# CVlab315/Domain-Adaptative-Hand-Pose-Estimation

Hardware: AMD Instinct MI355X
Metric: images/sec (unique source+target images per A+B+C training iteration, 2*B*N/t_iter) (higher is better)
Workload: dtype bf16; 1 GPU; RHD->H3D domain-adaptation iteration (steps A+B+C), resnet50 + 3-deconv neck + main head + 3 adversarial multiscale-fusion heads, 256x256, batch 64 source + 64 target per GPU, random init, synthetic batches; arch=resnet50, image_size=256, per_gpu_batch=64, global_batch=64, parallelism=dp1, hip_graphs=True, gradient_exchange=none (one rank)

## Files before the change

### domain-adaptative-hand-pose-estimation_amd/build.py

```python
import os
import re
import shutil
import subprocess
import sys
import tempfile
from concurrent.futures import ThreadPoolExecutor

HERE = os.path.dirname(os.path.abspath(__file__))
CSRC = os.path.join(HERE, 'csrc')
OUT = os.path.join(HERE, 'libmi355pose.so')
SOURCES = ['api.hip', 'igemm.hip', 'pgemm.hip', 'igemm_fp8.hip', 'mx_fp8.hip', 'wgrad_fp8.hip', 'bn.hip', 'pool_layout.hip', 'pw21.hip', 'heatmap.hip', 'optim.hip', 'augment.hip', 'teacher.hip', 'eval.hip', 'mmd.hip', 'jfa.hip', 'proto.hip', 'mixup.hip']
HEADERS = ['common.h', 'conv_plan.h', 'igemm_common.h', 'fp8_common.h', 'joint_pool.h', 'adam_slice.h']
HIPCC = os.environ.get('HIPCC', '/opt/rocm/bin/hipcc')
LLVM_BIN = os.environ.get('MI355_LLVM_BIN', '/opt/rocm/lib/llvm/bin')
FLAGS = ['--offload-arch=gfx950', '-O3', '-std=c++17', '-fPIC', '-Wall', '-Wno-unused-function',
         '-ffp-contract=off',
         '-fno-slp-vectorize']

_PK = re.compile(r'\bv_pk_[a-z0-9_]+_f32\b')
_OPSEL = re.compile(r'\bop_sel:\[([01,]+)\]')
_OPSEL_HI = re.compile(r'\bop_sel_hi:\[([01,]+)\]')


def _negated(flag):
    if flag.startswith('-fno-'):
        return '-f' + flag[5:]
# ... 132 lines not shown
```

### domain-adaptative-hand-pose-estimation_amd/csrc/conv_plan.h

```cpp
#pragma once
#include <stdlib.h>
#include "common.h"

#define MAX_TAPS 52
struct Tap { int8_t dy, dx; int16_t widx; };

struct Phase { int OHp, OWp, out_oy, out_ox, M, ntaps, tap0, ntm; };
struct GatherArgs {
  const void* A; const void* B; void* D;
  const float* bias; const void* residual; const float* scale;
  int Hi, Wi, Ci;
  int in_sy, in_sx;
  int Ho, Wo;
  int out_sy, out_sx;
  int Nout, ldb, ldd;
  int cshift;
  int accumulate;
  int nphase, ntn, ntiles;
  int hw;
  int lw;
  unsigned a_bytes, b_bytes;
  size_t stat_bytes;
  int stat_slices;
  const void* bnb_x; const void* bnb_y;
// ... 40 lines not shown
  bool stats256 = conv_knob("MI355_STATS_256", 1) != 0;
  int phases = (int)conv_knob("MI355_PHASES", 1);
  int wg_blocks = (int)conv_knob("MI355_WG_BLOCKS", 768);
  int wgrad_kw = (int)conv_knob("MI355_WGRAD_KW", 1);
  int wgrad_kw2 = (int)conv_knob("MI355_WGRAD_KW2", 1);
  bool wgrad_group256 = conv_knob("MI355_WGRAD_GROUP256", 1) != 0;
  bool wgrad_kw_group = conv_knob("MI355_WGRAD_KW_GROUP", 1) != 0;
  int wg_group_blocks = (int)conv_knob("MI355_WG_GROUP_BLOCKS", 512);
  int wg_group256_blocks = (int)conv_knob("MI355_WG_GROUP256_BLOCKS", 256);
  int wg_kw_group_blocks = (int)conv_knob("MI355_WG_KW_GROUP_BLOCKS", 512);
  int pgemm = (int)conv_knob("MI355_PGEMM", 1), pgemm_set = -1;
  int pg_add_maxk = (int)conv_knob("MI355_PG_ADD", 1) * 64;
  long pg_min_rows = conv_knob("MI355_PG_MIN_ROWS", 32768);
  int pg_ring = (int)conv_knob("MI355_PG_RING", 0), pg_bm = (int)conv_knob("MI355_PG_BM", 64);
  int pg_per_cu = (int)conv_knob("MI355_PG_PER_CU", 2);
  int fp8_tile = (int)conv_knob("MI355_FP8_TILE", -1);
  long fp8_kw3 = conv_knob("MI355_FP8_KW3", 1024), fp8_kw3_set = -1;
};
inline ConvKnobs& conv_knobs() { static ConvKnobs k; return k; }

static inline void describe_fwd(GatherArgs& a, const mi355_conv_desc* d) {
  a.Hi = d->Hi; a.Wi = d->Wi; a.Ci = d->Ci; a.in_sy = a.in_sx = d->stride;
  a.Ho = d->Ho; a.Wo = d->Wo; a.out_sy = a.out_sx = 1;
  a.Nout = d->Co; a.ldd = d->Co; a.ldb = d->kh * d->kw * d->Ci;
  a.nphase = 1; a.ph[0].OHp = d->Ho; a.ph[0].OWp = d->Wo; a.ph[0].M = d->N * d->Ho * d->Wo; a.ph[0].ntaps = d->kh * d->kw;
  for (int i = 0; i < d->kh; ++i)
    for (int j = 0; j < d->kw; ++j) { Tap& t = a.taps[i * d->kw + j]; t.dy = (int8_t)(i - d->pad); t.dx = (int8_t)(j - d->pad); t.widx = (int16_t)(i * d->kw + j); }
}
static inline bool describe_dgrad(GatherArgs& a, const mi355_conv_desc* d) {
  const int s = d->stride;
// ... 18 lines not shown
        for (int kw = 0; kw < d->kw; ++kw) {
          if ((px + d->pad - kw) % s != 0) continue;
          Tap& t = a.taps[nt++]; t.dy = (int8_t)((py + d->pad - kh) / s); t.dx = (int8_t)((px + d->pad - kw) / s);
          t.widx = (int16_t)(kh * d->kw + kw);
        }
      }
      P.ntaps = nt - P.tap0;
      if (P.ntaps == 0) continue;
      ++a.nphase;
    }
  return need_zero;
}
static inline bool dgrad_fuses_stats(const GatherArgs& a, int stride, bool need_zero) { return !need_zero && a.nphase == stride * stride; }
static inline size_t conv_stats_bytes(long rows, int C) { return (size_t)(rows / 64 + 8) * C * 3 * sizeof(float); }

enum ConvFamily { CONV_GATHER = 0, CONV_PGEMM, CONV_FP8, CONV_MX };
struct ConvBuild {
  int family = CONV_GATHER;
  int bm = 64, bn = 64;
  bool f32 = false;
  bool small_c = false;
  bool hm = false;
  bool dma = false;
  bool kw3 = false;
  bool cat = false;
  int kg = 1;
  int ns = 0; bool add = false;
  bool bf8 = false;
  int epi = 0;
};
static inline void conv_build_text(const ConvBuild& b, char* out, size_t n) {
  char epi[8] = "";
  if (b.epi) snprintf(epi, sizeof(epi), " epi%d", b.epi);
  if (b.family == CONV_PGEMM) snprintf(out, n, "pgemm bm%d bn%d ns%d%s%s", b.bm, b.bn, b.ns, epi, b.add ? " add" : "");
  else if (b.family == CONV_GATHER)
    snprintf(out, n, "%sg%dx%d%s%s%s%s%s%s%s", b.cat ? "cat " : "", b.bm, b.bn, b.f32 ? " f32" : "", b.small_c ? " small" : "", b.hm ? " hm" : "",
             b.dma ? " dma" : "", b.kw3 ? " kw3" : "", b.kg == 2 ? " kg2" : "", epi);
  else snprintf(out, n, "%s g%dx%d%s%s%s", b.family == CONV_MX ? "mx" : "f8", b.bm, b.bn, b.kw3 ? " kw3" : "", b.bf8 ? " bf8" : "", epi);
}

static inline bool kw3_shape(const GatherArgs& a) {
  if (!(a.nphase == 1 && a.ph[0].ntaps == 9 && a.in_sx == 1 && a.in_sy == 1 && a.out_sx == 1 && a.out_sy == 1 &&
        a.ph[0].OWp == a.Wi && a.ph[0].OHp == a.Hi && a.Wo == a.Wi && a.Ho == a.Hi && a.Wi >= 8 && a.Wi <= 128 && ilog2_exact(a.Wi) >= 0))
    return false;
  for (int g = 0; g < 3; ++g) {
    const Tap* tp = a.taps + a.ph[0].tap0 + 3 * g;
    int seen = 0;
    for (int k = 0; k < 3; ++k) { if (tp[k].dy != tp[0].dy || tp[k].dx < -1 || tp[k].dx > 1) return false; seen |= 1 << (tp[k].dx + 1); }
    if (seen != 7 || tp[0].dy < -1 || tp[0].dy > 1) return false;
// ... 89 lines not shown
  return b;
}
static inline int pgemm_plan_grid(GatherArgs& a, ConvBuild& b) {
  const int nk = a.Ci >> 6;
  a.pg_nadd = pgemm_nadd(b.ns, nk, b.add);
  const int smem = pgemm_smem(b.bm, b.bn, b.ns, nk, a.pg_nadd);
  if (smem > 160 * 1024) return 0;
  const int ntm = a.ph[0].ntm = cdiv(a.ph[0].M, b.bm);
  a.ntn = cdiv(a.Nout, b.bn);
  a.ntiles = ntm * a.ntn; a.stat_slices = 0;
  if (a.stat_partial && (b.add || (size_t)ntm * a.Nout * 3 * sizeof(float) > a.stat_bytes)) a.stat_partial = nullptr;
  b.epi = a.stat_partial ? 1 : 0;
  return smem;
}

static inline ConvBuild choose_conv(const GatherArgs& a, int elem_size, const ConvKnobs& k) {
  if (a.A2) return choose_cat(a, elem_size, k);
  const bool bf16 = elem_size == 2;
  if (bf16 && pgemm_eligible(a, 2, k)) return choose_pgemm(a, k);
  const GatherWork w = gather_work(a, elem_size);
  ConvBuild b;
  b.f32 = !bf16;
  if (w.small) { b.bm = 128; b.small_c = true; return b; }
  if (k.tile >= 0 && k.tile <= 3) {
    static const int forced[4][2] = {{128, 128}, {64, 128}, {128, 64}, {64, 64}};
    b.bm = forced[k.tile][0]; b.bn = forced[k.tile][1];
    return b;
  }
  const bool kw3 = k.kw3 && bf16 && kw3_shape(a) && (a.Nout > 64 || (k.kw3_n64 && a.Nout == 64)) && a.Ci % 64 == 0 && !a.bnb_partial;
  const long rows128 = cdiv(w.Mtot, 128L);
  if (a.Nout <= 64) {
    if (kw3 && (rows128 >= 2048 || k.kw3 == 2)) { b.bm = 128; b.kw3 = true; }
    else if (rows128 >= 512) b.bm = 128;
  }
// ... 178 lines not shown
```

### domain-adaptative-hand-pose-estimation_amd/csrc/igemm.hip

```cpp
#include "common.h"
#include <stdlib.h>

#include "igemm_common.h"

template <typename T> struct MmaTraits;
template <> struct MmaTraits<bf16_t> { static constexpr int BK = 64; static constexpr int CH = 8; };
template <> struct MmaTraits<float> { static constexpr int BK = 32; static constexpr int CH = 4; };

#define GATHER_STAGES 1
template <typename T, int BM, int BN, int STAGES = 1, bool KW3 = false>
struct GatherSmem {
  static constexpr int kARows = KW3 ? BM + 4 * (BM / 8) + 4 : BM;
  static constexpr int kStage = (kARows + BN) * 128;
  static constexpr int kOutStride = BN * (int)sizeof(T) + 16;
  static constexpr int kOut = BM * kOutStride;
  static constexpr int kBytes = (STAGES * kStage > kOut ? STAGES * kStage : kOut) + BM * 4;
};

template <typename T, int BM, int BN, bool SMALL_C, int WGM = 2, int WGN = 2, bool HM_OUT = false, bool DMA = false, int EPI = 0,
          bool KW3 = false, bool CAT = false, int KG = 1>
__global__ __launch_bounds__(64 * WGM * WGN * KG, (KW3 && BM == 256) ? 2 : 1) void gather_gemm_kernel(const GatherArgs p) {
  constexpr int CH = MmaTraits<T>::CH;
  constexpr int GTHR = 64 * WGM * WGN;
  constexpr int NTHR = GTHR * KG, RPP = GTHR / 8;
// ... 1308 lines not shown
    flops += 2.0 * a.ph[i].M * (double)a.Nout * a.ph[i].ntaps * a.Ci;
  }
  {
    const long imgs = a.ph[0].M / ((long)a.ph[0].OHp * a.ph[0].OWp);
    a.a_bytes = (unsigned)(imgs * a.Hi * a.Wi * a.Ci * (long)sizeof(T));
    a.b_bytes = (unsigned)((long)a.Nout * a.ldb * (long)sizeof(T));
  }
  if (a.A2) flops += 2.0 * Mtot * (double)a.Nout * a.c2;
  ProfScope ps(st, flops, (double)a.a_bytes + (double)a.b_bytes * ntaps_tot / (a.ldb / a.Ci) + (double)Mtot * a.Nout * sizeof(T) +
                              (a.A2 ? (double)a.a2_bytes + a.b2_bytes : 0.0));
  if (a.A2) {
    if ((a.Ci / CH) < 8 || a.nphase != 1 || a.out_sx != 1 || a.out_sy != 1 || a.bnb_partial || a.residual || a.accumulate)
      MI_FAIL(MI355_EINVAL, "concat-K forward: plain single-phase forward conv with >= 8 input chunks only");
    if (a.c2 < CH || a.c2 % CH || a.c2 > MmaTraits<T>::BK) MI_FAIL(MI355_EINVAL, "concat-K forward: c2=%d must be a multiple of %d and <= %d", a.c2, CH, MmaTraits<T>::BK);
  }
  const ConvBuild b = choose_conv(a, (int)sizeof(T), conv_knobs());
  if (b.family == CONV_PGEMM) return launch_pgemm_build(a, b, st);
  if (!launch_gather_build<T>(a, b, st)) MI_FAIL(MI355_EINVAL, "gather: no such build (%dx%d)", b.bm, b.bn);
  MI_CHECK_LAUNCH(b.cat ? "gather_gemm_cat" : "gather_gemm");
  return MI355_OK;
}

static int check_desc(const mi355_conv_desc* d, bool crop_ok = false) {
  if (!d) MI_FAIL(MI355_EINVAL, "null conv desc");
  if (d->dtype != MI355_F32 && d->dtype != MI355_BF16 && d->dtype != MI355_FP8) MI_FAIL(MI355_EINVAL, "bad dtype %d", d->dtype);
  if (d->kh * d->kw > MAX_TAPS || d->kh < 1 || d->kw < 1) MI_FAIL(MI355_EINVAL, "unsupported kernel %dx%d", d->kh, d->kw);
  if (d->stride < 1 || d->stride > 2) MI_FAIL(MI355_EINVAL, "unsupported stride %d", d->stride);
  const int fho = (d->Hi + 2 * d->pad - d->kh) / d->stride + 1, fwo = (d->Wi + 2 * d->pad - d->kw) / d->stride + 1;
  const bool cropped = crop_ok && d->stride == 1 && d->kh > 1 && d->dtype != MI355_FP8 && d->Ho >= 1 && d->Wo >= 1 && d->Ho <= fho && d->Wo <= fwo;
  if (!cropped && (d->Ho != fho || d->Wo != fwo))
    MI_FAIL(MI355_EINVAL, "conv desc: output size %dx%d inconsistent with input %dx%d k%d s%d p%d", d->Ho, d->Wo, d->Hi, d->Wi, d->kh, d->stride, d->pad);
  const long esz = d->dtype == MI355_F32 ? 4 : 2;
// ... 491 lines not shown
```

### domain-adaptative-hand-pose-estimation_amd/csrc/igemm_common.h

```cpp
#pragma once
#include "common.h"
#include "conv_plan.h"

template <typename T> __device__ __forceinline__ uint4 keep_masked(uint4 q, unsigned mb) {
  unsigned w[4] = {q.x, q.y, q.z, q.w};
  if constexpr (sizeof(T) == 2) {
#pragma unroll
    for (int i = 0; i < 4; ++i)
      w[i] &= ((0u - ((mb >> (2 * i)) & 1u)) & 0x0000ffffu) | ((0u - ((mb >> (2 * i + 1)) & 1u)) & 0xffff0000u);
  } else {
#pragma unroll
    for (int i = 0; i < 4; ++i) w[i] &= 0u - ((mb >> i) & 1u);
  }
  return make_uint4(w[0], w[1], w[2], w[3]);
}

__device__ __forceinline__ int swz128(int r, int c) { return r * 128 + ((c ^ ((r >> 1) & 7)) << 4); }

__device__ __forceinline__ int xcd_remap(int bid, int nblk) {
  int q = nblk >> 3, r = nblk & 7, x = bid & 7, i = bid >> 3;
  int start = (x < r) ? x * (q + 1) : r * (q + 1) + (x - r) * q;
  return start + i;
}

typedef __attribute__((ext_vector_type(4))) unsigned int u32x4_t;
#define OOB_OFF ((int)0x80000000)
__device__ __forceinline__ __amdgpu_buffer_rsrc_t make_rsrc(const void* p, unsigned bytes) {
  return __builtin_amdgcn_make_buffer_rsrc(const_cast<void*>(p), 0, bytes, 0x00020000);
}
__device__ __forceinline__ uint4 buf_load16(__amdgpu_buffer_rsrc_t rs, int byte_off) {
  u32x4_t v = __builtin_amdgcn_raw_buffer_load_b128(rs, byte_off, 0, 0);
  return make_uint4(v[0], v[1], v[2], v[3]);
}
__device__ __forceinline__ unsigned buf_load4(__amdgpu_buffer_rsrc_t rs, int byte_off) {
  return __builtin_amdgcn_raw_buffer_load_b32(rs, byte_off, 0, 0);
}


int launch_pgemm_build(GatherArgs& a, ConvBuild b, hipStream_t st);
int dispatch_gather_fp8(GatherArgs& a, hipStream_t st);

void launch_slab_reduce(const float* ws, float* dw, long n, int S, long stride, int accumulate, hipStream_t st);
```

### domain-adaptative-hand-pose-estimation_amd/csrc/pgemm.hip

```cpp
#include "common.h"
#include <stdlib.h>

#include "igemm_common.h"

template <int BM, int BN, int NS>
struct PgSmem {
  static constexpr int kStage = BM * 128;
  static constexpr int kOut = BM * BN * 2;
  static constexpr int bytes(int nk) { return nk * BN * 128 + NS * kStage + kOut; }
};

template <int BN> __device__ __forceinline__ int out_swz(int r, int c) {
  if constexpr (BN == 128) return r * 256 + ((c ^ (r & 15)) << 4);
  else return r * 128 + ((c ^ ((r >> 1) & 7)) << 4);
}

typedef __attribute__((address_space(3))) char* lds_cptr;
__device__ __forceinline__ unsigned lds_addr(const void* p) { return (unsigned)(uintptr_t)(lds_cptr)(const_cast<void*>(p)); }
__device__ __forceinline__ bf16x8_t lds_read16(unsigned a) { bf16x8_t v; asm volatile("ds_read_b128 %0, %1" : "=v"(v) : "v"(a)); return v; }
__device__ __forceinline__ u32x4_t lds_read16u(unsigned a) { u32x4_t v; asm volatile("ds_read_b128 %0, %1" : "=v"(v) : "v"(a)); return v; }
__device__ __forceinline__ void lds_write8(unsigned a, uint2 v) { asm volatile("ds_write_b64 %0, %1" :: "v"(a), "v"(v) : "memory"); }
__device__ __forceinline__ void lds_write4(unsigned a, float v) { asm volatile("ds_write_b32 %0, %1" :: "v"(a), "v"(v) : "memory"); }
__device__ __forceinline__ float lds_read4(unsigned a) { float v; asm volatile("ds_read_b32 %0, %1" : "=v"(v) : "v"(a)); return v; }
#define LDS_WAIT_ALL() asm volatile("s_waitcnt lgkmcnt(0)" ::: "memory")
#define RAW_BARRIER() asm volatile("s_barrier" ::: "memory")

template <int N> __device__ __forceinline__ void wait_vm() {
  static_assert(N >= 0, "vmcnt immediate");
  asm volatile("s_waitcnt vmcnt(%0)" :: "n"(N > 63 ? 63 : N) : "memory");
}
__device__ __forceinline__ void wait_vm_dyn(int a) {
  switch (a >> 1) {
    case 0: wait_vm<0>(); break;   case 1: wait_vm<2>(); break;   case 2: wait_vm<4>(); break;   case 3: wait_vm<6>(); break;
    case 4: wait_vm<8>(); break;   case 5: wait_vm<10>(); break;  case 6: wait_vm<12>(); break;  case 7: wait_vm<14>(); break;
    case 8: wait_vm<16>(); break;  case 9: wait_vm<18>(); break;  case 10: wait_vm<20>(); break; case 11: wait_vm<22>(); break;
    case 12: wait_vm<24>(); break; case 13: wait_vm<26>(); break; case 14: wait_vm<28>(); break; case 15: wait_vm<30>(); break;
    case 16: wait_vm<32>(); break; case 17: wait_vm<34>(); break; case 18: wait_vm<36>(); break; case 19: wait_vm<38>(); break;
    case 20: wait_vm<40>(); break; case 21: wait_vm<42>(); break; case 22: wait_vm<44>(); break; case 23: wait_vm<46>(); break;
    case 24: wait_vm<48>(); break; case 25: wait_vm<50>(); break; case 26: wait_vm<52>(); break; case 27: wait_vm<54>(); break;
    case 28: wait_vm<56>(); break; case 29: wait_vm<58>(); break; case 30: wait_vm<60>(); break; default: wait_vm<62>(); break;
  }
}

template <int BM, int BN, int NS, int EPI, bool ADD>
__global__ __launch_bounds__(256) void pgemm_kernel(const GatherArgs p) {
  constexpr int CH = 8, NTHR = 256;
  constexpr int WM = BM / 2, WN = BN / 2, MT = WM / 32, NT = WN / 32;
  constexpr int PA = BM / 32, PB = BN / 32;
  constexpr int DIST = NS - 1;
  constexpr int CPR = BN / CH;
  constexpr int IT = BM * CPR / NTHR;
  constexpr int RSTEP = NTHR / CPR;
  static_assert(BM * CPR % NTHR == 0, "whole passes only");
  using SM = PgSmem<BM, BN, NS>;
  extern __shared__ __attribute__((aligned(16))) char smem[];

  const int t = threadIdx.x, lane = t & 63, wave = t >> 6;
// ... 471 lines not shown
```

### domain-adaptative-hand-pose-estimation_amd/mi355/__init__.py

```python
import ctypes
import os
import threading

import torch

F32, BF16, FP8 = 0, 1, 2
_HERE = os.path.dirname(os.path.abspath(__file__))
LIB_PATH = os.environ.get('MI355_LIB') or os.path.join(os.path.dirname(_HERE), 'libmi355pose.so')

_lib = None
_lock = threading.Lock()


class Mi355Error(RuntimeError):
    pass


class ConvDesc(ctypes.Structure):
    _fields_ = [(n, ctypes.c_int) for n in
                ('N', 'Hi', 'Wi', 'Ci', 'Ho', 'Wo', 'Co', 'kh', 'kw', 'stride', 'pad', 'dtype')]


class WgradItem(ctypes.Structure):
    _fields_ = [('d', ConvDesc), ('x', ctypes.c_void_p), ('dy', ctypes.c_void_p), ('dw', ctypes.c_void_p),
# ... 40 lines not shown
    'mi355_pack_weights': (_I, [_P, _P, _P, _I, _I, _I, _I, _I, _P]),
    'mi355_pack_weights_batched': (_I, [_P, _I, _I, _I, _P]),
    'mi355_colsum_workspace': (_Z, [_L, _I]),
    'mi355_colsum': (_I, [_P, _P, _L, _I, _I, _I, _P, _Z, _P]),
    'mi355_bn_workspace': (_Z, [_L, _I]),
    'mi355_bn_train_fwd': (_I, [_P, _P, _P, _P, _P, _P, _P, _P, _P, _P, _L, _I, _F, _F, _I, _I, _I, _P, _Z, _P, _P, _P, _P]),
    'mi355_bn_train_fwd_partials': (_I, [_P, _P, _P, _P, _P, _P, _P, _P, _P, _P, _L, _I, _F, _F, _I, _I, _I, _P, _I, _P, _P, _P, _P, _P]),
    'mi355_bn_eval_fwd': (_I, [_P, _P, _P, _P, _P, _P, _P, _L, _I, _F, _I, _I, _P]),
    'mi355_bn_bwd_partials': (_I, [_P, _P, _P, _P, _P, _P, _P, _P, _P, _P, _P, _I, _L, _I, _I, _I, _P, _I, _P, _P, _P, _P, _P]),
    'mi355_bn_bwd': (_I, [_P, _P, _P, _P, _P, _P, _P, _P, _P, _P, _P, _I, _L, _I, _I, _I, _P, _Z, _P, _P, _P, _P]),
    'mi355_bn_resident_timeouts': (_I, [_P]),
    'mi355_bn_resident_reset': (_I, []),
    'mi355_bn_resident_set_spin_limit': (_I, [ctypes.c_uint]),
    'mi355_bn_set_resident': (_I, [_I]),
    'mi355_set_pgemm': (_I, [_I]),
    'mi355_set_fp8_kw3': (_L, [_L]),
    'mi355_apply_relu_mask': (_I, [_P, _P, _L, _I, _I, _P]),
    'mi355_conv_dgrad_masked_acc': (_I, [_P, _P, _P, _P, _P, _P, _P]),
    'mi355_conv_fwd_act': (_I, [_P, _P, _P, _P, _P, _I, _P, _P]),
    'mi355_conv_dgrad_act': (_I, [_P, _P, _P, _P, _I, _P, _P]),
    'mi355_bn_relu_maxpool_fwd_partials': (_I, [_P, _P, _P, _P, _P, _P, _P, _P, _P, _P, _I, _I, _I, _I, _F, _F, _I, _I, _P, _I, _P, _P]),
    'mi355_maxpool_fwd': (_I, [_P, _P, _P, _I, _I, _I, _I, _I, _P]),
    'mi355_maxpool_bwd': (_I, [_P, _P, _P, _I, _I, _I, _I, _I, _P]),
    'mi355_nchw_to_nhwc': (_I, [_P, _P, _I, _I, _I, _I, _I, _I, _P]),
    'mi355_nchw_to_s2d': (_I, [_P, _P, _I, _I, _I, _I, _P]),
    'mi355_stem_s2d_pack': (_I, [_P, _P, _I, _I, _P]),
    'mi355_stem_s2d_unpack_grad': (_I, [_P, _P, _I, _I, _P]),
    'mi355_nhwc_to_nchw': (_I, [_P, _P, _I, _I, _I, _I, _I, _P]),
    'mi355_conv1x1_heatmap': (_I, [_P, _P, _P, _P, _I, _I, _I, _I, _I, _P]),
    'mi355_pw_c2k': (_I, [_P, _P, _P, _P, _I, _I, _I, _I, _I, _I, _P]),
# ... 290 lines not shown
```

### include/mi355pose.h

```cpp
#ifndef MI355POSE_H
#define MI355POSE_H
#include <stddef.h>
#include <stdint.h>

#ifdef __cplusplus
extern "C" {
#endif

#define MI355_F32 0
#define MI355_BF16 1
#define MI355_FP8 2

#define MI355_OK 0
#define MI355_EINVAL (-1)
#define MI355_ELAUNCH (-2)
#define MI355_EWORKSPACE (-3)

typedef struct {
  int N, Hi, Wi, Ci;
  int Ho, Wo, Co;
  int kh, kw, stride, pad;
  int dtype;
} mi355_conv_desc;

int mi355_version(void);
const char* mi355_last_error(void);

int mi355_conv_fwd(const mi355_conv_desc* d, const void* x, const void* w, const float* bias,
                   const void* residual, void* y, void* stream);
int mi355_conv_dgrad(const mi355_conv_desc* d, const void* dy, const void* wT, const float* bias,
                     const float* scale_dev, int accumulate, void* dx, void* stream);
int mi355_set_pgemm(int mode);
int mi355_conv_fwd_act(const mi355_conv_desc* d, const void* x, const void* w, const float* bias, const void* residual, int relu,
                       void* y, void* stream);
int mi355_conv_dgrad_act(const mi355_conv_desc* d, const void* dy, const void* wT, const float* bias, int relu, void* dx,
                         void* stream);
int mi355_conv_dgrad_masked_acc(const mi355_conv_desc* d, const void* dy, const void* wT, const float* scale_dev, void* dx,
                                const void* acc_mask, void* stream);
size_t mi355_conv_stats_bytes(long rows, int C);
int mi355_conv_fwd_stats(const mi355_conv_desc* d, const void* x, const void* w, const float* bias, void* y,
                         float* partial, size_t partial_bytes, int* nslices, void* stream);
int mi355_conv_dgrad_stats(const mi355_conv_desc* d, const void* dy, const void* wT, void* dx, float* partial,
                           size_t partial_bytes, int* nslices, void* stream);
int mi355_conv_fwd_cat(const mi355_conv_desc* d, const void* x, const void* w, const float* bias, const void* x2,
                       const void* w2, const float* bias2, int c2, void* y, float* partial, size_t partial_bytes,
                       int* nslices, void* stream);
typedef struct mi355_bn_bwd_src {
// ... 237 lines not shown
```

### profiles/insitu_table.py

```python
import csv
import json
import re
import sys
import collections

trace, logf, iters = sys.argv[1], sys.argv[2], int(sys.argv[3])
MFMA, HBM = 1.75e15, 6.3e12

PAT = [('fwd8', 'gather_fp8_kernel'), ('dgrad8', 'gather_fp8_kernel'), ('fwd', ('gather_gemm_kernel', 'pgemm_kernel')),
       ('dgrad', ('gather_gemm_kernel', 'pgemm_kernel')), ('hm1x1', 'gather_gemm_kernel'), ('wgrad_kw_group', 'wgrad_kw_group_kernel'),
       ('wgrad_kw2', 'wgrad_kw2_kernel'), ('wgrad_kw', 'wgrad_kw_kernel'), ('wgrad_group256', 'wgrad_group256_kernel'), ('wgrad_group', 'wgrad_group_kernel'),
       ('wgrad8', 'wgrad_kw'), ('wgrad', 'wgrad_gemm_kernel'),
       ('bn_stats', 'bn_stats_kernel'), ('bn_finalize', 'bn_finalize'), ('bn_apply', 'bn_apply_kernel'), ('bn_relu_maxpool', 'bn_relu_maxpool_kernel'),
       ('bn_bwd_res', 'bn_bwd_resident_kernel'), ('bn_bwd_reduce', 'bn_bwd_reduce_kernel'), ('bn_bwd_finalize', 'bn_bwd_finalize_kernel'),
       ('bn_bwd_apply', 'bn_bwd_apply_kernel'), ('slab_reduce_group', 'slab_reduce_group_kernel'), ('slab_reduce', 'slab_reduce_kernel')]
FAMILY_KERNELS = {0: ('gather_gemm_kernel', 'gather_fp8_kernel', 'pgemm_kernel', 'wgrad_gemm_kernel', 'wgrad_kw_kernel', 'wgrad_kw2_kernel',
                      'wgrad_group_kernel', 'wgrad_group256_kernel', 'wgrad_kw_group_kernel', 'wgrad_kw8_kernel', 'wgrad_kw28_kernel'),
                  1: ('bn_stats_kernel', 'bn_finalize_kernel', 'bn_finalize_wide_kernel', 'bn_apply_kernel', 'bn_relu_maxpool_kernel',
                      'bn_bwd_resident_kernel', 'bn_bwd_reduce_kernel', 'bn_bwd_finalize_kernel', 'bn_bwd_apply_kernel'),
                  2: ('slab_reduce_kernel', 'slab_reduce_group_kernel')}


def base(name):
    m = re.match(r'_Z\d+([A-Za-z0-9_]+?)I', name)
    if m:
        return m.group(1)
    return re.sub(r'<.*|\(.*', '', re.sub(r'^void ', '', name)).strip()


log = json.load(open(logf))['launches']
rows = []
# ... 52 lines not shown
```

Measured before the change: 4358 images/s.

## Add weight-stationary persistent 3x3 conv kernel for 64-channel layers

Adds a persistent kernel for bf16 3x3 convolutions with 64 input and 64 output channels. It loads all nine weight taps into LDS once per block and streams 128-row activation tiles through a three-stage ring of async buffer-to-LDS loads, with optional fused BN statistics in the epilogue. The goal is to stop re-fetching weights on every tile and to overlap loads with MFMA work on the large layer1-sized convolutions. The cost is a large LDS footprint, which limits occupancy to roughly one block per CU, and a falls back to the gather path when the launch can't be planned.

```diff
diff --git a/domain-adaptative-hand-pose-estimation_amd/build.py b/domain-adaptative-hand-pose-estimation_amd/build.py
--- a/domain-adaptative-hand-pose-estimation_amd/build.py
+++ b/domain-adaptative-hand-pose-estimation_amd/build.py
@@ -9,7 +9,7 @@
 HERE = os.path.dirname(os.path.abspath(__file__))
 CSRC = os.path.join(HERE, 'csrc')
 OUT = os.path.join(HERE, 'libmi355pose.so')
-SOURCES = ['api.hip', 'igemm.hip', 'pgemm.hip', 'igemm_fp8.hip', 'mx_fp8.hip', 'wgrad_fp8.hip', 'bn.hip', 'pool_layout.hip', 'pw21.hip', 'heatmap.hip', 'optim.hip', 'augment.hip', 'teacher.hip', 'eval.hip', 'mmd.hip', 'jfa.hip', 'proto.hip', 'mixup.hip']
+SOURCES = ['api.hip', 'igemm.hip', 'pgemm.hip', 'ws3x3.hip', 'igemm_fp8.hip', 'mx_fp8.hip', 'wgrad_fp8.hip', 'bn.hip', 'pool_layout.hip', 'pw21.hip', 'heatmap.hip', 'optim.hip', 'augment.hip', 'teacher.hip', 'eval.hip', 'mmd.hip', 'jfa.hip', 'proto.hip', 'mixup.hip']
 HEADERS = ['common.h', 'conv_plan.h', 'igemm_common.h', 'fp8_common.h', 'joint_pool.h', 'adam_slice.h']
 HIPCC = os.environ.get('HIPCC', '/opt/rocm/bin/hipcc')
 LLVM_BIN = os.environ.get('MI355_LLVM_BIN', '/opt/rocm/lib/llvm/bin')
diff --git a/domain-adaptative-hand-pose-estimation_amd/csrc/conv_plan.h b/domain-adaptative-hand-pose-estimation_amd/csrc/conv_plan.h
--- a/domain-adaptative-hand-pose-estimation_amd/csrc/conv_plan.h
+++ b/domain-adaptative-hand-pose-estimation_amd/csrc/conv_plan.h
@@ -78,6 +78,8 @@
   long pg_min_rows = conv_knob("MI355_PG_MIN_ROWS", 32768);
   int pg_ring = (int)conv_knob("MI355_PG_RING", 0), pg_bm = (int)conv_knob("MI355_PG_BM", 64);
   int pg_per_cu = (int)conv_knob("MI355_PG_PER_CU", 2);
+  int ws3x3 = (int)conv_knob("MI355_WS3X3", 1), ws3x3_set = -1;
+  int ws3x3_grid = (int)conv_knob("MI355_WS3X3_GRID", 0);
   int fp8_tile = (int)conv_knob("MI355_FP8_TILE", -1);
   long fp8_kw3 = conv_knob("MI355_FP8_KW3", 1024), fp8_kw3_set = -1;
 };
@@ -126,7 +128,7 @@
 static inline bool dgrad_fuses_stats(const GatherArgs& a, int stride, bool need_zero) { return !need_zero && a.nphase == stride * stride; }
 static inline size_t conv_stats_bytes(long rows, int C) { return (size_t)(rows / 64 + 8) * C * 3 * sizeof(float); }
 
-enum ConvFamily { CONV_GATHER = 0, CONV_PGEMM, CONV_FP8, CONV_MX };
+enum ConvFamily { CONV_GATHER = 0, CONV_PGEMM, CONV_FP8, CONV_MX, CONV_WS3X3 };
 struct ConvBuild {
   int family = CONV_GATHER;
   int bm = 64, bn = 64;
@@ -145,6 +147,7 @@
   char epi[8] = "";
   if (b.epi) snprintf(epi, sizeof(epi), " epi%d", b.epi);
   if (b.family == CONV_PGEMM) snprintf(out, n, "pgemm bm%d bn%d ns%d%s%s", b.bm, b.bn, b.ns, epi, b.add ? " add" : "");
+  else if (b.family == CONV_WS3X3) snprintf(out, n, "ws3x3 bm%d ns%d%s", b.bm, b.ns, epi);
   else if (b.family == CONV_GATHER)
     snprintf(out, n, "%sg%dx%d%s%s%s%s%s%s%s", b.cat ? "cat " : "", b.bm, b.bn, b.f32 ? " f32" : "", b.small_c ? " small" : "", b.hm ? " hm" : "",
              b.dma ? " dma" : "", b.kw3 ? " kw3" : "", b.kg == 2 ? " kg2" : "", epi);
@@ -264,10 +267,51 @@
   return smem;
 }
 
+#define WS_BM 128
+#define WS_NS 3
+#define WS_THREADS 512
+constexpr int kWsARows = WS_BM + WS_BM / 8 + 2;
+constexpr int kWsStage = kWsARows * 128;
+constexpr int kWsWeights = 9 * 64 * 128;
+constexpr int kWsOut = WS_BM * 64 * 2;
+constexpr int kWsScratch = (WS_THREADS / 64) * 64 * 3 * 4;
+constexpr int kWsSmem = kWsWeights + WS_NS * kWsStage + kWsOut + kWsScratch;
+static_assert(kWsSmem <= 160 * 1024, "ws3x3: weights + ring + staging must fit one CU's LDS");
+static inline bool ws3x3_eligible(const GatherArgs& a, int elem_size, const ConvKnobs& k) {
+  const int mode = k.ws3x3_set >= 0 ? k.ws3x3_set : k.ws3x3;
+  if (!mode || elem_size != 2) return false;
+  if (a.A2 || a.Ci != 64 || a.Nout != 64 || a.ldb != 9 * 64 || a.ldd != 64) return false;
+  if (!kw3_shape(a) || a.ph[0].out_oy || a.ph[0].out_ox) return false;
+  if (a.residual || a.accumulate || a.acc_mask || a.scale || a.relu || a.bnb_partial || a.hw) return false;
+  const long Mrows = a.ph[0].M;
+  if (Mrows < 1 || (Mrows + 2L * a.Wi) * 128 >= (1L << 31)) return false;
+  if (mode >= 2) return true;
+  return k.kw3 && k.kw3_n64 && !(k.tile >= 0 && k.tile <= 3) && cdiv(Mrows, 128L) >= 2048;
+}
+static inline ConvBuild choose_ws3x3() {
+  ConvBuild b;
+  b.family = CONV_WS3X3; b.bm = WS_BM; b.bn = 64; b.ns = WS_NS;
+  return b;
+}
+static inline int ws3x3_plan_grid(GatherArgs& a, ConvBuild& b, int ncu, int per_cu, const ConvKnobs& k) {
+  if (ncu < 1 || per_cu < 1) return 0;
+  const int ntm = a.ph[0].ntm = cdiv(a.ph[0].M, WS_BM);
+  a.ntn = 1; a.ntiles = ntm; a.stat_slices = 0; a.lw = ilog2_exact(a.Wi);
+  if (a.stat_partial) {
+    if ((size_t)ntm * a.Nout * 3 * sizeof(float) <= a.stat_bytes) a.stat_slices = ntm;
+    else a.stat_partial = nullptr;
+  }
+  b.epi = a.stat_partial ? 1 : 0;
+  long grid = (long)ncu * per_cu;
+  if (k.ws3x3_grid > 0 && grid > k.ws3x3_grid) grid = k.ws3x3_grid;
+  return (int)(grid < ntm ? grid : ntm);
+}
+
 static inline ConvBuild choose_conv(const GatherArgs& a, int elem_size, const ConvKnobs& k) {
   if (a.A2) return choose_cat(a, elem_size, k);
   const bool bf16 = elem_size == 2;
   if (bf16 && pgemm_eligible(a, 2, k)) return choose_pgemm(a, k);
+  if (bf16 && ws3x3_eligible(a, 2, k)) return choose_ws3x3();
   const GatherWork w = gather_work(a, elem_size);
   ConvBuild b;
   b.f32 = !bf16;
diff --git a/domain-adaptative-hand-pose-estimation_amd/csrc/igemm.hip b/domain-adaptative-hand-pose-estimation_amd/csrc/igemm.hip
--- a/domain-adaptative-hand-pose-estimation_amd/csrc/igemm.hip
+++ b/domain-adaptative-hand-pose-estimation_amd/csrc/igemm.hip
@@ -1346,8 +1346,15 @@
       MI_FAIL(MI355_EINVAL, "concat-K forward: plain single-phase forward conv with >= 8 input chunks only");
     if (a.c2 < CH || a.c2 % CH || a.c2 > MmaTraits<T>::BK) MI_FAIL(MI355_EINVAL, "concat-K forward: c2=%d must be a multiple of %d and <= %d", a.c2, CH, MmaTraits<T>::BK);
   }
-  const ConvBuild b = choose_conv(a, (int)sizeof(T), conv_knobs());
+  ConvBuild b = choose_conv(a, (int)sizeof(T), conv_knobs());
   if (b.family == CONV_PGEMM) return launch_pgemm_build(a, b, st);
+  if (b.family == CONV_WS3X3) {
+    const int e = launch_ws3x3_build(a, b, st);
+    if (e <= 0) return e;
+    ConvKnobs without = conv_knobs();
+    without.ws3x3 = 0; without.ws3x3_set = 0;
+    b = choose_conv(a, (int)sizeof(T), without);
+  }
   if (!launch_gather_build<T>(a, b, st)) MI_FAIL(MI355_EINVAL, "gather: no such build (%dx%d)", b.bm, b.bn);
   MI_CHECK_LAUNCH(b.cat ? "gather_gemm_cat" : "gather_gemm");
   return MI355_OK;
diff --git a/domain-adaptative-hand-pose-estimation_amd/csrc/igemm_common.h b/domain-adaptative-hand-pose-estimation_amd/csrc/igemm_common.h
--- a/domain-adaptative-hand-pose-estimation_amd/csrc/igemm_common.h
+++ b/domain-adaptative-hand-pose-estimation_amd/csrc/igemm_common.h
@@ -36,8 +36,36 @@
   return __builtin_amdgcn_raw_buffer_load_b32(rs, byte_off, 0, 0);
 }
 
+typedef __attribute__((address_space(3))) char* lds_cptr;
+__device__ __forceinline__ unsigned lds_addr(const void* p) { return (unsigned)(uintptr_t)(lds_cptr)(const_cast<void*>(p)); }
+__device__ __forceinline__ bf16x8_t lds_read16(unsigned a) { bf16x8_t v; asm volatile("ds_read_b128 %0, %1" : "=v"(v) : "v"(a)); return v; }
+__device__ __forceinline__ u32x4_t lds_read16u(unsigned a) { u32x4_t v; asm volatile("ds_read_b128 %0, %1" : "=v"(v) : "v"(a)); return v; }
+__device__ __forceinline__ void lds_write8(unsigned a, uint2 v) { asm volatile("ds_write_b64 %0, %1" :: "v"(a), "v"(v) : "memory"); }
+__device__ __forceinline__ void lds_write4(unsigned a, float v) { asm volatile("ds_write_b32 %0, %1" :: "v"(a), "v"(v) : "memory"); }
+__device__ __forceinline__ float lds_read4(unsigned a) { float v; asm volatile("ds_read_b32 %0, %1" : "=v"(v) : "v"(a)); return v; }
+#define LDS_WAIT_ALL() asm volatile("s_waitcnt lgkmcnt(0)" ::: "memory")
+#define RAW_BARRIER() asm volatile("s_barrier" ::: "memory")
+
+template <int N> __device__ __forceinline__ void wait_vm() {
+  static_assert(N >= 0, "vmcnt immediate");
+  asm volatile("s_waitcnt vmcnt(%0)" :: "n"(N > 63 ? 63 : N) : "memory");
+}
+__device__ __forceinline__ void wait_vm_dyn(int a) {
+  switch (a >> 1) {
+    case 0: wait_vm<0>(); break;   case 1: wait_vm<2>(); break;   case 2: wait_vm<4>(); break;   case 3: wait_vm<6>(); break;
+    case 4: wait_vm<8>(); break;   case 5: wait_vm<10>(); break;  case 6: wait_vm<12>(); break;  case 7: wait_vm<14>(); break;
+    case 8: wait_vm<16>(); break;  case 9: wait_vm<18>(); break;  case 10: wait_vm<20>(); break; case 11: wait_vm<22>(); break;
+    case 12: wait_vm<24>(); break; case 13: wait_vm<26>(); break; case 14: wait_vm<28>(); break; case 15: wait_vm<30>(); break;
+    case 16: wait_vm<32>(); break; case 17: wait_vm<34>(); break; case 18: wait_vm<36>(); break; case 19: wait_vm<38>(); break;
+    case 20: wait_vm<40>(); break; case 21: wait_vm<42>(); break; case 22: wait_vm<44>(); break; case 23: wait_vm<46>(); break;
+    case 24: wait_vm<48>(); break; case 25: wait_vm<50>(); break; case 26: wait_vm<52>(); break; case 27: wait_vm<54>(); break;
+    case 28: wait_vm<56>(); break; case 29: wait_vm<58>(); break; case 30: wait_vm<60>(); break; default: wait_vm<62>(); break;
+  }
+}
+
 
 int launch_pgemm_build(GatherArgs& a, ConvBuild b, hipStream_t st);
+int launch_ws3x3_build(GatherArgs& a, ConvBuild b, hipStream_t st);
 int dispatch_gather_fp8(GatherArgs& a, hipStream_t st);
 
 void launch_slab_reduce(const float* ws, float* dw, long n, int S, long stride, int accumulate, hipStream_t st);
diff --git a/domain-adaptative-hand-pose-estimation_amd/csrc/pgemm.hip b/domain-adaptative-hand-pose-estimation_amd/csrc/pgemm.hip
--- a/domain-adaptative-hand-pose-estimation_amd/csrc/pgemm.hip
+++ b/domain-adaptative-hand-pose-estimation_amd/csrc/pgemm.hip
@@ -15,32 +15,6 @@
   else return r * 128 + ((c ^ ((r >> 1) & 7)) << 4);
 }
 
-typedef __attribute__((address_space(3))) char* lds_cptr;
-__device__ __forceinline__ unsigned lds_addr(const void* p) { return (unsigned)(uintptr_t)(lds_cptr)(const_cast<void*>(p)); }
-__device__ __forceinline__ bf16x8_t lds_read16(unsigned a) { bf16x8_t v; asm volatile("ds_read_b128 %0, %1" : "=v"(v) : "v"(a)); return v; }
-__device__ __forceinline__ u32x4_t lds_read16u(unsigned a) { u32x4_t v; asm volatile("ds_read_b128 %0, %1" : "=v"(v) : "v"(a)); return v; }
-__device__ __forceinline__ void lds_write8(unsigned a, uint2 v) { asm volatile("ds_write_b64 %0, %1" :: "v"(a), "v"(v) : "memory"); }
-__device__ __forceinline__ void lds_write4(unsigned a, float v) { asm volatile("ds_write_b32 %0, %1" :: "v"(a), "v"(v) : "memory"); }
-__device__ __forceinline__ float lds_read4(unsigned a) { float v; asm volatile("ds_read_b32 %0, %1" : "=v"(v) : "v"(a)); return v; }
-#define LDS_WAIT_ALL() asm volatile("s_waitcnt lgkmcnt(0)" ::: "memory")
-#define RAW_BARRIER() asm volatile("s_barrier" ::: "memory")
-
-template <int N> __device__ __forceinline__ void wait_vm() {
-  static_assert(N >= 0, "vmcnt immediate");
-  asm volatile("s_waitcnt vmcnt(%0)" :: "n"(N > 63 ? 63 : N) : "memory");
-}
-__device__ __forceinline__ void wait_vm_dyn(int a) {
-  switch (a >> 1) {
-    case 0: wait_vm<0>(); break;   case 1: wait_vm<2>(); break;   case 2: wait_vm<4>(); break;   case 3: wait_vm<6>(); break;
-    case 4: wait_vm<8>(); break;   case 5: wait_vm<10>(); break;  case 6: wait_vm<12>(); break;  case 7: wait_vm<14>(); break;
-    case 8: wait_vm<16>(); break;  case 9: wait_vm<18>(); break;  case 10: wait_vm<20>(); break; case 11: wait_vm<22>(); break;
-    case 12: wait_vm<24>(); break; case 13: wait_vm<26>(); break; case 14: wait_vm<28>(); break; case 15: wait_vm<30>(); break;
-    case 16: wait_vm<32>(); break; case 17: wait_vm<34>(); break; case 18: wait_vm<36>(); break; case 19: wait_vm<38>(); break;
-    case 20: wait_vm<40>(); break; case 21: wait_vm<42>(); break; case 22: wait_vm<44>(); break; case 23: wait_vm<46>(); break;
-    case 24: wait_vm<48>(); break; case 25: wait_vm<50>(); break; case 26: wait_vm<52>(); break; case 27: wait_vm<54>(); break;
-    case 28: wait_vm<56>(); break; case 29: wait_vm<58>(); break; case 30: wait_vm<60>(); break; default: wait_vm<62>(); break;
-  }
-}
 
 template <int BM, int BN, int NS, int EPI, bool ADD>
 __global__ __launch_bounds__(256) void pgemm_kernel(const GatherArgs p) {
diff --git a/domain-adaptative-hand-pose-estimation_amd/csrc/ws3x3.hip b/domain-adaptative-hand-pose-estimation_amd/csrc/ws3x3.hip
--- /dev/null
+++ b/domain-adaptative-hand-pose-estimation_amd/csrc/ws3x3.hip
@@ -0,0 +1,321 @@
+#include "common.h"
+#include <stdlib.h>
+
+#include "igemm_common.h"
+
+__device__ __forceinline__ void lds_write16z(unsigned a) {
+  const u32x4_t z = {0u, 0u, 0u, 0u};
+  asm volatile("ds_write_b128 %0, %1" :: "v"(a), "v"(z) : "memory");
+}
+__device__ __forceinline__ uint2 lds_read8(unsigned a) { uint2 v; asm volatile("ds_read_b64 %0, %1" : "=v"(v) : "v"(a)); return v; }
+__device__ __forceinline__ float lane_read(unsigned lane_byte, float v) {
+  float r; asm volatile("ds_bpermute_b32 %0, %1, %2" : "=v"(r) : "v"(lane_byte), "v"(v)); return r;
+}
+
+template <int EPI>
+__global__ __launch_bounds__(WS_THREADS) void ws3x3_kernel(const GatherArgs p) {
+  constexpr int BM = WS_BM, NTHR = WS_THREADS;
+  constexpr bool stats = EPI == 1;
+  constexpr int IT = stats ? 4 : 2;
+  static_assert(WS_NS == 3, "stage g of a tile lives in ring slot g");
+  extern __shared__ __attribute__((aligned(16))) char smem[];
+
+  const int t = threadIdx.x, lane = t & 63, wave = t >> 6;
+  const int wave_u = __builtin_amdgcn_readfirstlane(wave);
+  const int r31 = lane & 31, hi = lane >> 5;
+  const int wm0 = (wave >> 1) * 32, wn0 = (wave & 1) * 32;
+  const int lc = lane & 7, lr8 = lane >> 3;
+  const int M = p.ph[0].M, ntm = p.ph[0].ntm, lw = p.lw, W = p.Wi, H = p.Hi;
+  const int G = (int)gridDim.x;
+  const int b0 = xcd_remap((int)blockIdx.x, G);
+  const int my_tiles = b0 < ntm ? (ntm - b0 + G - 1) / G : 0;
+  if (my_tiles == 0) return;
+  const unsigned smem_base = lds_addr(smem);
+  const unsigned ring_base = smem_base + (unsigned)kWsWeights, out_base = ring_base + (unsigned)(WS_NS * kWsStage);
+  const unsigned scr_base = out_base + (unsigned)kWsOut;
+  (void)scr_base;
+
+  const Tap* __restrict__ ptaps = p.taps + p.ph[0].tap0;
+  int dxs[9], wix[9], dys[3];
+#pragma unroll
+  for (int i = 0; i < 9; ++i) { dxs[i] = ptaps[i].dx; wix[i] = ptaps[i].widx; }
+#pragma unroll
+  for (int g = 0; g < 3; ++g) dys[g] = ptaps[3 * g].dy;
+#pragma unroll
+  for (int i = 0; i < 9; ++i) asm volatile("" : "+s"(dxs[i]), "+s"(wix[i]));
+#pragma unroll
+  for (int g = 0; g < 3; ++g) asm volatile("" : "+s"(dys[g]));
+
+  {
+    const int nz = ((BM >> lw) + 1) * 8;
+    for (int i = t; i < WS_NS * nz; i += NTHR) {
+      const int st = i / nz, rem = i - st * nz;
+      lds_write16z(ring_base + (unsigned)(st * kWsStage + (rem >> 3) * (W + 1) * 128 + (rem & 7) * 16));
+    }
+    LDS_WAIT_ALL();
+  }
+  float4 bq[4];
+#pragma unroll
+  for (int g = 0; g < 4; ++g) {
+    bq[g] = p.bias ? *reinterpret_cast<const float4*>(p.bias + wn0 + 8 * g + 4 * hi) : make_float4(0.f, 0.f, 0.f, 0.f);
+    asm volatile("" : "+v"(bq[g].x), "+v"(bq[g].y), "+v"(bq[g].z), "+v"(bq[g].w));
+  }
+
+  const __amdgpu_buffer_rsrc_t rsA = make_rsrc(p.A, p.a_bytes), rsB = make_rsrc(p.B, p.b_bytes);
+  (void)rsA; (void)rsB;
+  {
+    const int n = wave * 8 + lr8, lcs = lc ^ ((n >> 1) & 7);
+    (void)n; (void)lcs;
+#if defined(__HIP_DEVICE_COMPILE__)
+    typedef __attribute__((address_space(3))) void* ldsp;
+#pragma unroll
+    for (int i = 0; i < 9; ++i)
+      __builtin_amdgcn_raw_ptr_buffer_load_lds(rsB, (ldsp)(smem + i * 8192 + wave_u * 1024), 16, (n * p.ldb + lcs * 8) * 2, wix[i] * 128, 0, 0);
+#endif
+  }
+  int dst_off[2], lane_off[2], qrow[2];
+#pragma unroll
+  for (int j = 0; j < 2; ++j) {
+    const int q0 = (wave_u + 8 * j) * 8, q = q0 + lr8, R = 1 + q + (q >> lw);
+    dst_off[j] = (1 + q0 + (q0 >> lw)) * 128;
+    lane_off[j] = q * 128 + ((lc ^ ((R >> 1) & 7)) << 4);
+    qrow[j] = q;
+  }
+  int voff[2], ym[2];
+  auto set_issue_tile = [&](int i) {
+    const int m0 = (b0 + i * G) * BM;
+#pragma unroll
+    for (int j = 0; j < 2; ++j) {
+      const int m = m0 + qrow[j];
+      ym[j] = m < M ? (int)(((unsigned)m >> lw) % (unsigned)H) : -(1 << 20);
+      voff[j] = m0 * 128 + lane_off[j];
+    }
+  };
+  auto issue = [&](int g) {
+    const int dy = dys[g];
+    (void)dy;
+#if defined(__HIP_DEVICE_COMPILE__)
+    typedef __attribute__((address_space(3))) void* ldsp;
+#pragma unroll
+    for (int j = 0; j < 2; ++j) {
+      const bool ok = (unsigned)(ym[j] + dy) < (unsigned)H;
+      __builtin_amdgcn_raw_ptr_buffer_load_lds(rsA, (ldsp)(smem + kWsWeights + g * kWsStage + dst_off[j]), 16,
+                                               ok ? voff[j] + dy * W * 128 : OOB_OFF, 0, 0, 0);
+    }
+#endif
+  };
+
+  const int rimg = 1 + (wm0 + r31) + ((wm0 + r31) >> lw);
+  unsigned fb[4];
+#pragma unroll
+  for (int s = 0; s < 4; ++s) fb[s] = (unsigned)swz128(wn0 + r31, 2 * s + hi);
+  f32x16_t acc;
+#define WS_RD(DA, AA, DB, AB, OFF) "ds_read_b128 " DA ", " AA "\n\tds_read_b128 " DB ", " AB " offset:" #OFF "\n"
+#define WS_MM(B, A) "v_mfma_f32_32x32x16_bf16 %[acc], " B ", " A ", %[acc]\n"
+#define WS_W2 "s_waitcnt lgkmcnt(2)\n"
+  auto compute = [&](int g) {
+    unsigned xa[3][4], xb[4];
+#pragma unroll
+    for (int kw = 0; kw < 3; ++kw) {
+      const int r = rimg + dxs[3 * g + kw];
+      const unsigned row = ring_base + (unsigned)(g * kWsStage + r * 128), x = (unsigned)((r >> 1) & 7);
+#pragma unroll
+      for (int s = 0; s < 4; ++s) xa[kw][s] = row + (((unsigned)(2 * s + hi) ^ x) << 4);
+    }
+#pragma unroll
+    for (int s = 0; s < 4; ++s) xb[s] = smem_base + (unsigned)(3 * g * 8192) + fb[s];
+    bf16x8_t a0, b0, a1, b1;
+    asm volatile(
+        WS_RD("%[a0]", "%[x00]", "%[b0]", "%[y0]", 0) WS_RD("%[a1]", "%[x01]", "%[b1]", "%[y1]", 0)
+        WS_W2 WS_MM("%[b0]", "%[a0]") WS_RD("%[a0]", "%[x02]", "%[b0]", "%[y2]", 0)
+        WS_W2 WS_MM("%[b1]", "%[a1]") WS_RD("%[a1]", "%[x03]", "%[b1]", "%[y3]", 0)
+        WS_W2 WS_MM("%[b0]", "%[a0]") WS_RD("%[a0]", "%[x10]", "%[b0]", "%[y0]", 8192)
+        WS_W2 WS_MM("%[b1]", "%[a1]") WS_RD("%[a1]", "%[x11]", "%[b1]", "%[y1]", 8192)
+        WS_W2 WS_MM("%[b0]", "%[a0]") WS_RD("%[a0]", "%[x12]", "%[b0]", "%[y2]", 8192)
+        WS_W2 WS_MM("%[b1]", "%[a1]") WS_RD("%[a1]", "%[x13]", "%[b1]", "%[y3]", 8192)
+        WS_W2 WS_MM("%[b0]", "%[a0]") WS_RD("%[a0]", "%[x20]", "%[b0]", "%[y0]", 16384)
+        WS_W2 WS_MM("%[b1]", "%[a1]") WS_RD("%[a1]", "%[x21]", "%[b1]", "%[y1]", 16384)
+        WS_W2 WS_MM("%[b0]", "%[a0]") WS_RD("%[a0]", "%[x22]", "%[b0]", "%[y2]", 16384)
+        WS_W2 WS_MM("%[b1]", "%[a1]") WS_RD("%[a1]", "%[x23]", "%[b1]", "%[y3]", 16384)
+        WS_W2 WS_MM("%[b0]", "%[a0]")
+        "s_waitcnt lgkmcnt(0)\n" WS_MM("%[b1]", "%[a1]")
+        : [acc] "+v"(acc), [a0] "=&v"(a0), [b0] "=&v"(b0), [a1] "=&v"(a1), [b1] "=&v"(b1)
+        : [x00] "v"(xa[0][0]), [x01] "v"(xa[0][1]), [x02] "v"(xa[0][2]), [x03] "v"(xa[0][3]),
+          [x10] "v"(xa[1][0]), [x11] "v"(xa[1][1]), [x12] "v"(xa[1][2]), [x13] "v"(xa[1][3]),
+          [x20] "v"(xa[2][0]), [x21] "v"(xa[2][1]), [x22] "v"(xa[2][2]), [x23] "v"(xa[2][3]),
+          [y0] "v"(xb[0]), [y1] "v"(xb[1]), [y2] "v"(xb[2]), [y3] "v"(xb[3])
+        : "memory");
+  };
+#undef WS_RD
+#undef WS_MM
+#undef WS_W2
+
+  unsigned so[4];
+#pragma unroll
+  for (int g = 0; g < 4; ++g) { const int nl = wn0 + 8 * g + 4 * hi, r = wm0 + r31; so[g] = (unsigned)(r * 128 + (((nl >> 3) ^ ((r >> 1) & 7)) << 4) + (nl & 7) * 2); }
+  bf16_t* __restrict__ D = reinterpret_cast<bf16_t*>(p.D);
+  auto epilogue = [&](int tm) {
+    const int m0 = tm * BM;
+    asm volatile("s_nop 7\n\ts_nop 7\n\ts_nop 3" : "+v"(acc) :: "memory");
+#pragma unroll
+    for (int g = 0; g < 4; ++g) {
+      const float bb[4] = {bq[g].x, bq[g].y, bq[g].z, bq[g].w};
+      union { bf16_t h[4]; uint2 q; } u;
+#pragma unroll
+      for (int e = 0; e < 4; ++e) u.h[e] = (bf16_t)(acc[4 * g + e] + bb[e]);
+      lds_write8(out_base + so[g], u.q);
+    }
+    LDS_WAIT_ALL();
+    RAW_BARRIER();
+    if constexpr (!stats) {
+      const int ec = t & 7, er = t >> 3;
+      const unsigned rd = out_base + (unsigned)(er * 128 + ((ec ^ ((er >> 1) & 7)) << 4));
+      u32x4_t q[2];
+#pragma unroll
+      for (int k = 0; k < 2; ++k) q[k] = lds_read16u(rd + (unsigned)(k * 64 * 128));
+      asm volatile("s_waitcnt lgkmcnt(0)" : "+v"(q[0]), "+v"(q[1]));
+#pragma unroll
+      for (int k = 0; k < 2; ++k) {
+        const int m = m0 + er + 64 * k;
+        if (m < M) *reinterpret_cast<uint4*>(D + (size_t)m * 64 + ec * 8) = make_uint4(q[k][0], q[k][1], q[k][2], q[k][3]);
+      }
+    } else {
+      const int vt = t >> 1, hf = t & 1, sc = vt & 7, sr = vt >> 3;
+      const unsigned rd = out_base + (unsigned)(sr * 128 + ((sc ^ ((sr >> 1) & 7)) << 4) + hf * 8);
+      uint2 q[4];
+#pragma unroll
+      for (int k = 0; k < 4; ++k) q[k] = lds_read8(rd + (unsigned)(k * 32 * 128));
+      asm volatile("s_waitcnt lgkmcnt(0)" : "+v"(q[0]), "+v"(q[1]), "+v"(q[2]), "+v"(q[3]));
+      float sn = 0.f, smean[4], sm2[4];
+#pragma unroll
+      for (int e = 0; e < 4; ++e) { smean[e] = 0.f; sm2[e] = 0.f; }
+#pragma unroll
+      for (int k = 0; k < 4; ++k) {
+        const int m = m0 + sr + 32 * k;
+        if (m >= M) continue;
+        const float v[4] = {__uint_as_float(q[k].x << 16), __uint_as_float(q[k].x & 0xffff0000u),
+                            __uint_as_float(q[k].y << 16), __uint_as_float(q[k].y & 0xffff0000u)};
+        sn += 1.f; const float inv = 1.f / sn;
+#pragma unroll
+        for (int e = 0; e < 4; ++e) { const float d = v[e] - smean[e]; smean[e] += d * inv; sm2[e] += d * (v[e] - smean[e]); }
+        *reinterpret_cast<uint2*>(D + (size_t)m * 64 + sc * 8 + hf * 4) = q[k];
+      }
+#pragma unroll
+      for (int o = 16; o < 64; o <<= 1) {
+        const unsigned src = (unsigned)(((lane + o) & 63) * 4);
+        float nb = lane_read(src, sn), mb[4], vb[4];
+#pragma unroll
+        for (int e = 0; e < 4; ++e) { mb[e] = lane_read(src, smean[e]); vb[e] = lane_read(src, sm2[e]); }
+        asm volatile("s_waitcnt lgkmcnt(0)" : "+v"(nb), "+v"(mb[0]), "+v"(mb[1]), "+v"(mb[2]), "+v"(mb[3]), "+v"(vb[0]), "+v"(vb[1]), "+v"(vb[2]), "+v"(vb[3]));
+        const float nt = sn + nb, f = nt > 0.f ? nb / nt : 0.f;
+#pragma unroll
+        for (int e = 0; e < 4; ++e) { const float d = mb[e] - smean[e]; smean[e] += d * f; sm2[e] += vb[e] + d * d * sn * f; }
+        sn = nt;
+      }
+      if (lane < 16) {
+#pragma unroll
+        for (int e = 0; e < 4; ++e) {
+          const unsigned qa = scr_base + (unsigned)(((wave * 64 + sc * 8 + hf * 4 + e) * 3) * 4);
+          lds_write4(qa, sn); lds_write4(qa + 4, smean[e]); lds_write4(qa + 8, sm2[e]);
+        }
+      }
+      LDS_WAIT_ALL();
+      RAW_BARRIER();
+      if (t < 64) {
+        float qn[8], qm[8], qv[8];
+#pragma unroll
+        for (int w = 0; w < 8; ++w) {
+          const unsigned qa = scr_base + (unsigned)(((w * 64 + t) * 3) * 4);
+          qn[w] = lds_read4(qa); qm[w] = lds_read4(qa + 4); qv[w] = lds_read4(qa + 8);
+        }
+        asm volatile("s_waitcnt lgkmcnt(0)" : "+v"(qn[0]), "+v"(qn[1]), "+v"(qn[2]), "+v"(qn[3]), "+v"(qn[4]), "+v"(qn[5]), "+v"(qn[6]), "+v"(qn[7]));
+        asm volatile("" : "+v"(qm[0]), "+v"(qm[1]), "+v"(qm[2]), "+v"(qm[3]), "+v"(qm[4]), "+v"(qm[5]), "+v"(qm[6]), "+v"(qm[7]));
+        asm volatile("" : "+v"(qv[0]), "+v"(qv[1]), "+v"(qv[2]), "+v"(qv[3]), "+v"(qv[4]), "+v"(qv[5]), "+v"(qv[6]), "+v"(qv[7]));
+        float cn = 0.f, mean = 0.f, m2 = 0.f;
+#pragma unroll
+        for (int vw = 0; vw < 4; ++vw) {
+          float wn = qn[2 * vw], wmean = qm[2 * vw], wm2 = qv[2 * vw];
+          {
+            const float nb = qn[2 * vw + 1], nt = wn + nb, f = nt > 0.f ? nb / nt : 0.f;
+            const float d = qm[2 * vw + 1] - wmean;
+            wmean += d * f; wm2 += qv[2 * vw + 1] + d * d * wn * f;
+            wn = nt;
+          }
+          if (wn > 0.f) { const float nt = cn + wn, f = wn / nt, d = wmean - mean; mean += d * f; m2 += wm2 + d * d * cn * f; cn = nt; }
+        }
+        float* out = p.stat_partial + ((size_t)tm * 64 + t) * 3;
+        out[0] = cn; out[1] = mean; out[2] = m2;
+      }
+    }
+  };
+
+  set_issue_tile(0);
+  issue(0); issue(1);
+  for (int ti = 0; ti < my_tiles; ++ti) {
+    const bool more = ti + 1 < my_tiles;
+#pragma unroll
+    for (int r = 0; r < 16; ++r) acc[r] = 0.f;
+#pragma unroll
+    for (int g = 0; g < 3; ++g) {
+#if defined(__HIP_DEVICE_COMPILE__)
+      if (g < 2) { if (ti > 0) wait_vm<2 + IT>(); else wait_vm<2>(); }
+      else { if (more) wait_vm<2>(); else wait_vm<0>(); }
+#endif
+      RAW_BARRIER();
+      if (g == 0) issue(2);
+      else if (more) { if (g == 1) set_issue_tile(ti + 1); issue(g - 1); }
+      __builtin_amdgcn_s_setprio(1);
+      compute(g);
+      __builtin_amdgcn_s_setprio(0);
+    }
+    epilogue(b0 + ti * G);
+  }
+}
+
+template <int EPI>
+static int ws3x3_blocks_per_cu() {
+  static int per_cu = -1;
+  if (per_cu < 0) {
+    auto kern = ws3x3_kernel<EPI>;
+    int nb = 0;
+    if (hipFuncSetAttribute((const void*)kern, hipFuncAttributeMaxDynamicSharedMemorySize, kWsSmem) != hipSuccess ||
+        hipOccupancyMaxActiveBlocksPerMultiprocessor(&nb, kern, WS_THREADS, (size_t)kWsSmem) != hipSuccess || nb < 1) nb = 0;
+    (void)hipGetLastError();
+    per_cu = nb;
+  }
+  return per_cu;
+}
+template <int EPI>
+static void launch_ws3x3_epi(const GatherArgs& a, const ConvBuild& b, int grid, hipStream_t st) {
+  if (prof_on()) { char text[64]; conv_build_text(b, text, sizeof(text)); prof_amend_label("[%s]", text); }
+  hipLaunchKernelGGL(ws3x3_kernel<EPI>, dim3(grid), dim3(WS_THREADS), kWsSmem, st, a);
+}
+
+extern "C" int mi355_set_ws3x3(int mode) {
+  const int prev = conv_knobs().ws3x3_set;
+  conv_knobs().ws3x3_set = mode < 0 ? -1 : (mode > 2 ? 2 : mode);
+  return prev;
+}
+extern "C" int mi355_set_ws3x3_grid(int max_blocks) {
+  const int prev = conv_knobs().ws3x3_grid;
+  conv_knobs().ws3x3_grid = max_blocks < 0 ? 0 : max_blocks;
+  return prev;
+}
+
+int launch_ws3x3_build(GatherArgs& a, ConvBuild b, hipStream_t st) {
+  static int ncu = 0;
+  if (!ncu) {
+    int dev = 0, v = 0;
+    if (hipGetDevice(&dev) != hipSuccess || hipDeviceGetAttribute(&v, hipDeviceAttributeMultiprocessorCount, dev) != hipSuccess || v < 1) return 1;
+    ncu = v;
+  }
+  const bool want_stats = a.stat_partial != nullptr && (size_t)cdiv(a.ph[0].M, WS_BM) * a.Nout * 3 * sizeof(float) <= a.stat_bytes;
+  const int per_cu = want_stats ? ws3x3_blocks_per_cu<1>() : ws3x3_blocks_per_cu<0>();
+  if (per_cu < 1) return 1;
+  const int grid = ws3x3_plan_grid(a, b, ncu, per_cu, conv_knobs());
+  if (grid < 1) return 1;
+  if (b.epi == 1) launch_ws3x3_epi<1>(a, b, grid, st);
+  else launch_ws3x3_epi<0>(a, b, grid, st);
+  MI_CHECK_LAUNCH("ws3x3");
+  return MI355_OK;
+}
diff --git a/domain-adaptative-hand-pose-estimation_amd/mi355/__init__.py b/domain-adaptative-hand-pose-estimation_amd/mi355/__init__.py
--- a/domain-adaptative-hand-pose-estimation_amd/mi355/__init__.py
+++ b/domain-adaptative-hand-pose-estimation_amd/mi355/__init__.py
@@ -78,6 +78,8 @@
     'mi355_bn_resident_set_spin_limit': (_I, [ctypes.c_uint]),
     'mi355_bn_set_resident': (_I, [_I]),
     'mi355_set_pgemm': (_I, [_I]),
+    'mi355_set_ws3x3': (_I, [_I]),
+    'mi355_set_ws3x3_grid': (_I, [_I]),
     'mi355_set_fp8_kw3': (_L, [_L]),
     'mi355_apply_relu_mask': (_I, [_P, _P, _L, _I, _I, _P]),
     'mi355_conv_dgrad_masked_acc': (_I, [_P, _P, _P, _P, _P, _P, _P]),
diff --git a/include/mi355pose.h b/include/mi355pose.h
--- a/include/mi355pose.h
+++ b/include/mi355pose.h
@@ -31,6 +31,8 @@
 int mi355_conv_dgrad(const mi355_conv_desc* d, const void* dy, const void* wT, const float* bias,
                      const float* scale_dev, int accumulate, void* dx, void* stream);
 int mi355_set_pgemm(int mode);
+int mi355_set_ws3x3(int mode);
+int mi355_set_ws3x3_grid(int max_blocks);
 int mi355_conv_fwd_act(const mi355_conv_desc* d, const void* x, const void* w, const float* bias, const void* residual, int relu,
                        void* y, void* stream);
 int mi355_conv_dgrad_act(const mi355_conv_desc* d, const void* dy, const void* wT, const float* bias, int relu, void* dx,
diff --git a/profiles/insitu_table.py b/profiles/insitu_table.py
--- a/profiles/insitu_table.py
+++ b/profiles/insitu_table.py
@@ -7,14 +7,14 @@
 trace, logf, iters = sys.argv[1], sys.argv[2], int(sys.argv[3])
 MFMA, HBM = 1.75e15, 6.3e12
 
-PAT = [('fwd8', 'gather_fp8_kernel'), ('dgrad8', 'gather_fp8_kernel'), ('fwd', ('gather_gemm_kernel', 'pgemm_kernel')),
-       ('dgrad', ('gather_gemm_kernel', 'pgemm_kernel')), ('hm1x1', 'gather_gemm_kernel'), ('wgrad_kw_group', 'wgrad_kw_group_kernel'),
+PAT = [('fwd8', 'gather_fp8_kernel'), ('dgrad8', 'gather_fp8_kernel'), ('fwd', ('gather_gemm_kernel', 'pgemm_kernel', 'ws3x3_kernel')),
+       ('dgrad', ('gather_gemm_kernel', 'pgemm_kernel', 'ws3x3_kernel')), ('hm1x1', 'gather_gemm_kernel'), ('wgrad_kw_group', 'wgrad_kw_group_kernel'),
        ('wgrad_kw2', 'wgrad_kw2_kernel'), ('wgrad_kw', 'wgrad_kw_kernel'), ('wgrad_group256', 'wgrad_group256_kernel'), ('wgrad_group', 'wgrad_group_kernel'),
        ('wgrad8', 'wgrad_kw'), ('wgrad', 'wgrad_gemm_kernel'),
        ('bn_stats', 'bn_stats_kernel'), ('bn_finalize', 'bn_finalize'), ('bn_apply', 'bn_apply_kernel'), ('bn_relu_maxpool', 'bn_relu_maxpool_kernel'),
        ('bn_bwd_res', 'bn_bwd_resident_kernel'), ('bn_bwd_reduce', 'bn_bwd_reduce_kernel'), ('bn_bwd_finalize', 'bn_bwd_finalize_kernel'),
        ('bn_bwd_apply', 'bn_bwd_apply_kernel'), ('slab_reduce_group', 'slab_reduce_group_kernel'), ('slab_reduce', 'slab_reduce_kernel')]
-FAMILY_KERNELS = {0: ('gather_gemm_kernel', 'gather_fp8_kernel', 'pgemm_kernel', 'wgrad_gemm_kernel', 'wgrad_kw_kernel', 'wgrad_kw2_kernel',
+FAMILY_KERNELS = {0: ('gather_gemm_kernel', 'gather_fp8_kernel', 'pgemm_kernel', 'ws3x3_kernel', 'wgrad_gemm_kernel', 'wgrad_kw_kernel', 'wgrad_kw2_kernel',
                       'wgrad_group_kernel', 'wgrad_group256_kernel', 'wgrad_kw_group_kernel', 'wgrad_kw8_kernel', 'wgrad_kw28_kernel'),
                   1: ('bn_stats_kernel', 'bn_finalize_kernel', 'bn_finalize_wide_kernel', 'bn_apply_kernel', 'bn_relu_maxpool_kernel',
                       'bn_bwd_resident_kernel', 'bn_bwd_reduce_kernel', 'bn_bwd_finalize_kernel', 'bn_bwd_apply_kernel'),
```

After: 4363 images/s (median of 4 runs). No clear change (+0.1%).
